# dedis/kyber

Measured on AMD Instinct MI355X. Metric: scalar-muls/s + pairings/s per node; MSM sec at 2^20 points, higher is better.
Workload: dtype int32 limbs (radix 2^25.5), int64 accumulate; 1 GPU; Ed25519 batched fixed-base + var-base scalar-mul, 2^20 scalars per GPU (BASELINE.json configs[1]); elements_per_gpu=1048576

## Files before the change

kyber_amd/csrc/ed25519.hip:

```cpp
#ifndef KYB_TU_WAVES
#define KYB_TU_WAVES 2
#endif
#include "context.h"
#include "ed25519_dev.cuh"
#include "msm.cuh"
#include "ed25519_h2c.cuh"
#include <stdlib.h>
#include <string.h>

#include <algorithm>
#include <atomic>
#include <chrono>
#include <thread>
#include <vector>

namespace kyb {


template <int G = 2>
__global__ void ed25519_build_base_table_kernel(int32_t* __restrict__ tab, const uint32_t* __restrict__ point,
                                                uint32_t* __restrict__ ok, int rows = ED_TAB_POS * ED_TAB_ENT) {
    const int t = blockIdx.x * blockDim.x + threadIdx.x;
    if (t >= rows) return;
    ge_p3 B;
    if (point) {
        uint32_t pw[8];
        load_words8(pw, point);
        const bool good = ge_p3_fromwords(B, pw);
        if (t == 0) *ok = good ? 1u : 0u;
    } else {
        B.X = fe_bx(); B.Y = fe_by(); fe_1(B.Z); B.T = fe_bt();
    }
    ed_comb_row<G>(tab + (size_t)t * ED_TAB_STRIDE, t, B);
}

__global__ __launch_bounds__(64, KYB_TU_WAVES) void ed25519_encode_kernel(size_t n, const int32_t* __restrict__ proj,
                                                            const uint8_t* __restrict__ status,
                                                            uint32_t* __restrict__ out) {
    ed_encode_chunk(n, proj, (size_t)blockIdx.x * blockDim.x + threadIdx.x, [&](size_t i, uint32_t (&w)[8]) {
        if (status && status[i]) {
#pragma unroll
            for (int k = 0; k < 8; k++) w[k] = 0;
        }
        store_words8(out + i * 8, w);
    });
}


template <int G>
__global__ __launch_bounds__(256, 3) void ed25519_mul_base_kernel(
    size_t n, const uint32_t* __restrict__ scalars, uint32_t* __restrict__ out,
    const int32_t* __restrict__ tab, uint32_t flags, int32_t* __restrict__ proj) {
    const bool full = (flags & KYB_F_VARTIME) != 0;
    for (size_t idx = (size_t)blockIdx.x * blockDim.x + threadIdx.x; idx < n;
         idx += (size_t)gridDim.x * blockDim.x) {
        uint32_t a[8];
        load_words8(a, scalars + idx * 8);
        int8_t e[65];
        recode16(e, a, full);
        ge_p3 h;
        ge_p3_0(h);
        ge_precomp t;
        ge_p1p1 r;
        const int npos = full ? EdComb<G>::POS : EdComb<G>::POS_CT;
#pragma unroll 1
        for (int k = 0; k < npos; k++) {
            int d = 0;
#pragma unroll
            for (int i = G - 1; i >= 0; i--)
                if (G * k + i <= 64) d = 16 * d + (int)e[G * k + i];
            if (full && __ballot(d != 0) == 0) continue;
            select_precomp_tab<EdComb<G>::ENT>(t, tab, k, d);
            ge_madd(r, h, t);
            ge_p1p1_to_p3(h, r);
        }
        if (proj) {
            store_proj(proj, idx, h);
            continue;
        }
        uint32_t w[8];
        ge_p3_towords(w, h);
        store_words8(out + idx * 8, w);
    }
}

KYB_DEV void select_precomp_uniform(ge_precomp& t, const int32_t* __restrict__ tab, int i, int b) {
    const bool neg = b < 0;
    const int babs = neg ? -b : b;
    const int pos = i >> 1, mult = (i & 1) ? 16 : 1;
    fe_1(t.ypx);
    fe_1(t.ymx);
    fe_0(t.xy2d);
#pragma unroll 1
    for (int m = 1; m <= 8; m++) {
        const int4* e = reinterpret_cast<const int4*>(tab + (size_t)(pos * ED_TAB_ENT + (m * mult - 1)) * ED_TAB_STRIDE);
        int32_t w[32];
#pragma unroll
        for (int q = 0; q < 8; q++) {
            const int4 x = e[q];
            w[4 * q] = x.x;
            w[4 * q + 1] = x.y;
            w[4 * q + 2] = x.z;
            w[4 * q + 3] = x.w;
        }
        const int32_t keep = -(int32_t)(babs == m);
#pragma unroll
        for (int l = 0; l < 10; l++) {
            t.ypx.v[l] ^= (t.ypx.v[l] ^ w[l]) & keep;
            t.ymx.v[l] ^= (t.ymx.v[l] ^ w[10 + l]) & keep;
            t.xy2d.v[l] ^= (t.xy2d.v[l] ^ w[20 + l]) & keep;
        }
    }
    ge_precomp_cneg(t, neg);
}
__global__ __launch_bounds__(256, 3) void ed25519_mul_base_uniform_kernel(
    size_t n, const uint32_t* __restrict__ scalars, uint32_t* __restrict__ out,
    const int32_t* __restrict__ tab, int32_t* __restrict__ proj) {
    for (size_t idx = (size_t)blockIdx.x * blockDim.x + threadIdx.x; idx < n;
         idx += (size_t)gridDim.x * blockDim.x) {
        uint32_t a[8];
        load_words8(a, scalars + idx * 8);
        int8_t e[65];
        recode16(e, a, false);
        ge_p3 h;
        ge_p3_0(h);
        ge_precomp t;
        ge_p1p1 r;
#pragma unroll 1
        for (int i = 0; i < 64; i++) {
            select_precomp_uniform(t, tab, i, (int)e[i]);
            ge_madd(r, h, t);
            ge_p1p1_to_p3(h, r);
        }
        if (proj) {
            store_proj(proj, idx, h);
            continue;
        }
        uint32_t w[8];
        ge_p3_towords(w, h);
        store_words8(out + idx * 8, w);
    }
}


template <bool GTAB, bool UNI = false>
__global__ __launch_bounds__(128, 3) void ed25519_mul_kernel(
    size_t n, const uint32_t* __restrict__ scalars, const uint32_t* __restrict__ points,
    size_t points_stride, uint32_t* __restrict__ out, uint8_t* __restrict__ status,
    uint32_t flags, int32_t* __restrict__ proj, int4* __restrict__ gtab) {
    const size_t idx = (size_t)blockIdx.x * blockDim.x + threadIdx.x;
    if (idx >= n) return;
    const bool full = !UNI && (flags & KYB_F_VARTIME) != 0;
    uint32_t pw[8], a[8];
    load_words8(pw, points + idx * points_stride);
    load_words8(a, scalars + idx * 8);
    ge_p3 A;
    const bool ok = ge_p3_fromwords(A, pw);
    int8_t e[65];
    recode16(e, a, full);
    ge_p3 h;
    const int vt_top = full ? wave_top_digit(a) : 63;
    if constexpr (GTAB) {
        TabGlobal tab{gtab + idx * 80};
        ge_scalarmult_w4<UNI>(h, e, A, full, tab, vt_top);
    } else {
        TabScratch tab;
        ge_scalarmult_w4<UNI>(h, e, A, full, tab, vt_top);
    }
    if (proj) {
        store_proj(proj, idx, h);
        if (status) status[idx] = ok ? KYB_ST_OK : KYB_ST_BAD_POINT;
        return;
    }
    uint32_t w[8];
    ge_p3_towords(w, h);
    if (!ok) {
#pragma unroll
        for (int i = 0; i < 8; i++) w[i] = 0;
    }
    store_words8(out + idx * 8, w);
    if (status) status[idx] = ok ? KYB_ST_OK : KYB_ST_BAD_POINT;
}

int ed25519_build_tables(DeviceCtx* ctx) {
    KYB_HIP_CHECK(hipMalloc(&ctx->ed_base_tab, ED_TAB_WORDS * sizeof(int32_t)));
    hipLaunchKernelGGL(ed25519_build_base_table_kernel<2>, dim3((ED_TAB_POS * ED_TAB_ENT + 63) / 64), dim3(64), 0,
                       nullptr, ctx->ed_base_tab, (const uint32_t*)nullptr, (uint32_t*)nullptr, ED_TAB_POS * ED_TAB_ENT);
    KYB_HIP_CHECK(hipGetLastError());
    const auto t0 = std::chrono::steady_clock::now();
    KYB_HIP_CHECK(hipMalloc(&ctx->ed_wide_tab, ED_WIDE_WORDS * sizeof(int32_t)));
    hipLaunchKernelGGL(ed25519_build_base_table_kernel<ED_COMB_G>, dim3((EdWide::ROWS + 63) / 64), dim3(64), 0, nullptr,
                       ctx->ed_wide_tab, (const uint32_t*)nullptr, (uint32_t*)nullptr, EdWide::ROWS);
    KYB_HIP_CHECK(hipGetLastError());
    KYB_HIP_CHECK(hipStreamSynchronize(nullptr));
    ctx->ed_wide_build_us = std::chrono::duration_cast<std::chrono::microseconds>(std::chrono::steady_clock::now() - t0).count();
    return KYB_OK;
}
void ed25519_free_tables(DeviceCtx* ctx) {
    if (ctx->ed_base_tab) hipFree(ctx->ed_base_tab);
    if (ctx->ed_wide_tab) hipFree(ctx->ed_wide_tab);
    ctx->ed_base_tab = ctx->ed_wide_tab = nullptr;
}

constexpr size_t ENC_DEFER_MIN = 4096;

static int ed_proj_workspace(DeviceCtx* ctx, hipStream_t st, size_t n, bool need_status, int32_t** proj,
                             uint8_t** status, int4** gtab = nullptr) {
    const size_t tab_bytes = gtab ? n * 1280 : 0;
    const size_t want = tab_bytes + n * 30 * sizeof(int32_t) + (need_status ? n : 0) + 256;
    void* base;
    int rc = ctx_workspace(ctx, WS_ED, st, want, &base);
    if (rc) return rc;
    if (gtab) *gtab = (int4*)base;
    *proj = (int32_t*)((uint8_t*)base + tab_bytes);
    if (status) *status = (uint8_t*)base + tab_bytes + n * 30 * sizeof(int32_t);
    return KYB_OK;
}

static int launch_mul_base(DeviceCtx* ctx, size_t n, const void* d_scalars, void* d_out, uint32_t flags,
                           hipStream_t st, const int32_t* tab = nullptr) {
    const bool wide = !tab && !(flags & KYB_F_UNIFORM);
    if (!tab) tab = wide ? ctx->ed_wide_tab : ctx->ed_base_tab;
    if (n == 0) return KYB_OK;
    const int block = 256;
    size_t want = (n + block - 1) / block;
    size_t cap = (size_t)ctx->num_cu * 8;
    int grid = (int)(want < cap ? want : cap);
    int32_t* proj = nullptr;
    std::lock_guard<std::recursive_mutex> enq_lock(ctx->enq_mu);
    if (n >= ENC_DEFER_MIN) {
        int rc = ed_proj_workspace(ctx, st, n, false, &proj, nullptr);
        if (rc) return rc;
    }
    if (flags & KYB_F_UNIFORM)
        hipLaunchKernelGGL(ed25519_mul_base_uniform_kernel, dim3(grid), dim3(block), 0, st, n,
                           (const uint32_t*)d_scalars, (uint32_t*)d_out, tab, proj);
    else if (wide)
        hipLaunchKernelGGL(ed25519_mul_base_kernel<ED_COMB_G>, dim3(grid), dim3(block), 0, st, n,
                           (const uint32_t*)d_scalars, (uint32_t*)d_out, tab, flags, proj);
    else
        hipLaunchKernelGGL(ed25519_mul_base_kernel<2>, dim3(grid), dim3(block), 0, st, n,
                           (const uint32_t*)d_scalars, (uint32_t*)d_out, tab, flags, proj);
    if (proj) {
        const size_t lanes = (n + ENC_CHUNK - 1) / ENC_CHUNK;
        hipLaunchKernelGGL(ed25519_encode_kernel, dim3((unsigned)((lanes + 63) / 64)), dim3(64), 0, st, n, proj,
                           (const uint8_t*)nullptr, (uint32_t*)d_out);
    }
    KYB_HIP_CHECK(hipGetLastError());
    return KYB_OK;
}
static int launch_mul(size_t n, const void* d_scalars, const void* d_points, size_t stride, void* d_out,
                      void* d_status, uint32_t flags, hipStream_t st) {
    if (n == 0) return KYB_OK;
    const int block = 128;
    size_t grid = (n + block - 1) / block;
    int32_t* proj = nullptr;
    int4* gtab = nullptr;
    uint8_t* stat = (uint8_t*)d_status;
    DeviceCtx* ctx;
    int rc = get_ctx(&ctx);
    if (rc) return rc;
    std::lock_guard<std::recursive_mutex> enq_lock(ctx->enq_mu);
    if (n >= ENC_DEFER_MIN) {
        rc = ed_proj_workspace(ctx, st, n, stat == nullptr, &proj, stat ? nullptr : &stat, &gtab);
        if (rc) return rc;
        if (flags & KYB_F_UNIFORM)
            hipLaunchKernelGGL((ed25519_mul_kernel<true, true>), dim3((unsigned)grid), dim3(block), 0, st, n,
                               (const uint32_t*)d_scalars, (const uint32_t*)d_points, stride, (uint32_t*)d_out, stat, flags,
                               proj, gtab);
        else
            hipLaunchKernelGGL(ed25519_mul_kernel<true>, dim3((unsigned)grid), dim3(block), 0, st, n,
                               (const uint32_t*)d_scalars, (const uint32_t*)d_points, stride, (uint32_t*)d_out, stat, flags,
                               proj, gtab);
    } else if (flags & KYB_F_UNIFORM) {
        hipLaunchKernelGGL((ed25519_mul_kernel<false, true>), dim3((unsigned)grid), dim3(block), 0, st, n,
                           (const uint32_t*)d_scalars, (const uint32_t*)d_points, stride, (uint32_t*)d_out, stat, flags,
                           proj, gtab);
    } else {
        hipLaunchKernelGGL(ed25519_mul_kernel<false>, dim3((unsigned)grid), dim3(block), 0, st, n,
                           (const uint32_t*)d_scalars, (const uint32_t*)d_points, stride, (uint32_t*)d_out, stat, flags,
                           proj, gtab);
    }
    if (proj) {
        const size_t lanes = (n + ENC_CHUNK - 1) / ENC_CHUNK;
        hipLaunchKernelGGL(ed25519_encode_kernel, dim3((unsigned)((lanes + 63) / 64)), dim3(64), 0, st, n, proj,
                           (const uint8_t*)stat, (uint32_t*)d_out);
    }
    KYB_HIP_CHECK(hipGetLastError());
    return KYB_OK;
}

}

using namespace kyb;

static bool ed_mul_flags_bad(uint32_t flags) {
    return (flags & ~(KYB_F_VARTIME | KYB_F_UNIFORM)) || (flags & (KYB_F_VARTIME | KYB_F_UNIFORM)) == (KYB_F_VARTIME | KYB_F_UNIFORM);
}

extern "C" {

int kyb_ed25519_mul_base_dev(size_t n, const void* d_scalars, void* d_out, uint32_t flags, void* stream) {
    if ((n && (!d_scalars || !d_out)) || ed_mul_flags_bad(flags)) {
        set_error("kyb_ed25519_mul_base_dev: bad argument");
        return KYB_E_ARG;
    }
    DeviceCtx* ctx;
    int rc = get_ctx(&ctx);
    if (rc) return rc;
    return launch_mul_base(ctx, n, d_scalars, d_out, flags, (hipStream_t)stream);
}

int kyb_ed25519_mul_dev(size_t n, const void* d_scalars, const void* d_points, void* d_out, void* d_status,
                        uint32_t flags, void* stream) {
    if ((n && (!d_scalars || !d_points || !d_out)) || ed_mul_flags_bad(flags)) {
        set_error("kyb_ed25519_mul_dev: bad argument");
        return KYB_E_ARG;
    }
    DeviceCtx* ctx;
    int rc = get_ctx(&ctx);
    if (rc) return rc;
    return launch_mul(n, d_scalars, d_points, 8, d_out, d_status, flags, (hipStream_t)stream);
}

static int mul_host(size_t n, const uint8_t* scalars, const uint8_t* points, size_t stride, uint8_t* out,
                    uint8_t* status, uint32_t flags);

int kyb_ed25519_mul_base(size_t n, const uint8_t* scalars, uint8_t* out, uint32_t flags) {
    if ((n && (!scalars || !out)) || ed_mul_flags_bad(flags)) {
        set_error("kyb_ed25519_mul_base: bad argument");
        return KYB_E_ARG;
    }
    if (n == 0) return KYB_OK;
    if (md_active(n))
        return md_run(n, [&](int, size_t lo, size_t hi) { return kyb_ed25519_mul_base(hi - lo, scalars + 32 * lo, out + 32 * lo, flags); });
    return mul_host(n, scalars, nullptr, 0, out, nullptr, flags);
}

constexpr size_t PIPE_CHUNK_MAX = PIN_SLOT_ELEMS;
constexpr int PIPE_SLOTS = DeviceCtx::NPIN, PIPE_STREAMS = 3;
static size_t pipe_chunk(const DeviceCtx* ctx) {
    if (const char* e = getenv("KYB_PIPE_CHUNK")) {
        const size_t v = (size_t)strtoull(e, nullptr, 10) & ~size_t(63);
        if (v >= 4096) return std::min(PIPE_CHUNK_MAX, v);
    }
    (void)ctx;
    return size_t(1) << 17;
}
static int pipe_nstreams() {
    if (const char* e = getenv("KYB_PIPE_STREAMS")) {
        const int v = atoi(e);
        if (v >= 1 && v <= PIPE_STREAMS) return v;
    }
    return 2;
}
constexpr size_t SAME_BASE_TABLE_MIN = 16384;

static int pipe_streams(DeviceCtx::StagePool* pool) {
    for (int i = 0; i < PIPE_STREAMS; i++)
        if (!pool->pipe[i]) KYB_HIP_CHECK(hipStreamCreateWithFlags(&pool->pipe[i], hipStreamNonBlocking));
    return KYB_OK;
}

static int mul_host(size_t n, const uint8_t* scalars, const uint8_t* points, size_t stride, uint8_t* out,
                    uint8_t* status, uint32_t flags) {
    DeviceCtx* ctx;
    int rc = get_ctx(&ctx);
    if (rc) return rc;
    bool fixed = points == nullptr;
    const size_t npts = fixed ? 0 : (stride ? n : 1);
    StageScope sc_(ctx);
    StageBuf d_s, d_p, d_o, d_st, d_tab;
    if ((rc = d_s.alloc(n * 32))) return rc;
    if ((rc = d_p.alloc(npts * 32))) return rc;
    if ((rc = d_o.alloc(n * 32))) return rc;
    if ((rc = d_st.alloc(n))) return rc;
    const int32_t* tab = nullptr;
    if (!fixed && !stride && (n >= SAME_BASE_TABLE_MIN || (flags & KYB_F_UNIFORM))) {
        if ((rc = d_tab.alloc(ED_TAB_WORDS * sizeof(int32_t) + 256))) return rc;
        uint32_t* d_ok = (uint32_t*)((uint8_t*)d_tab.p + ED_TAB_WORDS * sizeof(int32_t));
        KYB_HIP_CHECK(hipMemcpy(d_p.p, points, 32, hipMemcpyHostToDevice));
        hipLaunchKernelGGL(ed25519_build_base_table_kernel<2>, dim3((ED_TAB_POS * ED_TAB_ENT + 63) / 64), dim3(64), 0, sc_.stream(),
                           (int32_t*)d_tab.p, (const uint32_t*)d_p.p, d_ok, ED_TAB_POS * ED_TAB_ENT);
        uint32_t ok = 0;
        KYB_HIP_CHECK(hipMemcpy(&ok, d_ok, 4, hipMemcpyDeviceToHost));
        if (!ok) {
            memset(out, 0, n * 32);
            if (status) memset(status, KYB_ST_BAD_POINT, n);
            return KYB_OK;
        }
        if (status) memset(status, 0, n);
        tab = (const int32_t*)d_tab.p;
        fixed = true;
    }
    auto launch = [&](size_t off, size_t cnt, hipStream_t st) -> int {
        uint8_t* s = (uint8_t*)d_s.p + off * 32;
        uint8_t* o = (uint8_t*)d_o.p + off * 32;
        if (fixed) return launch_mul_base(ctx, cnt, s, o, flags, st, tab);
        const uint8_t* p = (const uint8_t*)d_p.p + (stride ? off * 32 : 0);
        return launch_mul(cnt, s, p, stride, o, (uint8_t*)d_st.p + off, flags, st);
    };
    const size_t PIPE_CHUNK = pipe_chunk(ctx);
    if (n < 2 * PIPE_CHUNK) {
        KYB_HIP_CHECK(hipMemcpy(d_s.p, scalars, n * 32, hipMemcpyHostToDevice));
        if (npts) KYB_HIP_CHECK(hipMemcpy(d_p.p, points, npts * 32, hipMemcpyHostToDevice));
        if ((rc = launch(0, n, nullptr))) return rc;
        if ((rc = d_o.download(out, n * 32))) return rc;
        if (status && !fixed) rc = d_st.download(status, n);
        return rc;
    }
    DeviceCtx::StagePool* pool = sc_.pool;
    if ((rc = pipe_streams(pool))) return rc;
    const int nstreams = pipe_nstreams();
    const bool per_point = !fixed && stride;
    const bool want_status = status && !fixed;
    if ((rc = ctx_pin_slots(pool))) return rc;
    const size_t nchunks = (n + PIPE_CHUNK - 1) / PIPE_CHUNK;
    std::vector<hipEvent_t> ev_out(nchunks);
    for (size_t i = 0; i < nchunks; i++) KYB_HIP_CHECK(hipEventCreateWithFlags(&ev_out[i], hipEventDisableTiming));
    auto enqueue = [&](size_t i) -> int {
        const size_t off = i * PIPE_CHUNK, cnt = std::min(PIPE_CHUNK, n - off);
        uint8_t* pin = (uint8_t*)pool->pin_in[i % PIPE_SLOTS];
        uint8_t* pout = (uint8_t*)pool->pin_out[i % PIPE_SLOTS];
        hipStream_t s_k = pool->pipe[i % nstreams];
        par_memcpy(pin, scalars + off * 32, cnt * 32);
        if (per_point) par_memcpy(pin + PIPE_CHUNK_MAX * 32, points + off * 32, cnt * 32);
        int r;
        if (fixed) {
            r = launch_mul_base(ctx, cnt, pin, pout, flags, s_k, tab);
        } else {
            const uint8_t* p = per_point ? pin + PIPE_CHUNK_MAX * 32 : (const uint8_t*)d_p.p;
            r = launch_mul(cnt, pin, p, stride, pout, (uint8_t*)d_st.p + off, flags, s_k);
        }
        if (r) return r;
        if (want_status)
            KYB_HIP_CHECK(hipMemcpyAsync(pout + PIPE_CHUNK_MAX * 32, (uint8_t*)d_st.p + off, cnt, hipMemcpyDeviceToHost, s_k));
        KYB_HIP_CHECK(hipEventRecord(ev_out[i], s_k));
        return KYB_OK;
    };
    auto drain = [&](size_t i) -> int {
        const size_t off = i * PIPE_CHUNK, cnt = std::min(PIPE_CHUNK, n - off);
        KYB_HIP_CHECK(hipEventSynchronize(ev_out[i]));
        const uint8_t* pout = (const uint8_t*)pool->pin_out[i % PIPE_SLOTS];
        par_memcpy(out + off * 32, pout, cnt * 32);
        if (want_status) memcpy(status + off, pout + PIPE_CHUNK_MAX * 32, cnt);
        return KYB_OK;
    };
    if (!fixed && !stride) KYB_HIP_CHECK(hipMemcpy(d_p.p, points, 32, hipMemcpyHostToDevice));
    std::atomic<size_t> enqueued{0}, drained{0};
    std::atomic<int> drain_rc{KYB_OK};
    std::atomic<bool> stop{false};
    const int device = ctx->device;
    std::string drain_err;
    std::thread drainer([&] {
        if (hipSetDevice(device) != hipSuccess) {
            drain_err = "ed25519 host pipeline: hipSetDevice failed on the drain thread";
            drain_rc.store(KYB_E_HIP);
            return;
        }
        for (size_t i = 0; i < nchunks; i++) {
            while (enqueued.load(std::memory_order_acquire) <= i) {
                if (stop.load(std::memory_order_acquire)) return;
                std::this_thread::yield();
            }
            const int r = drain(i);
            if (r) {
                drain_err = kyb_last_error();
                drain_rc.store(r);
                return;
            }
            drained.store(i + 1, std::memory_order_release);
        }
    });
    for (size_t i = 0; i < nchunks && rc == KYB_OK; i++) {
        while (i >= (size_t)PIPE_SLOTS && drained.load(std::memory_order_acquire) + PIPE_SLOTS <= i && drain_rc.load() == KYB_OK)
            std::this_thread::yield();
        if (drain_rc.load() != KYB_OK) break;
        rc = enqueue(i);
        if (rc == KYB_OK) enqueued.store(i + 1, std::memory_order_release);
    }
    if (rc != KYB_OK) stop.store(true, std::memory_order_release);
    drainer.join();
    if (rc == KYB_OK && (rc = drain_rc.load()) != KYB_OK) set_error(drain_err);
    hipError_t e2 = hipSuccess;
    for (int i = 0; i < PIPE_STREAMS; i++) {
        const hipError_t e = hipStreamSynchronize(pool->pipe[i]);
        if (e != hipSuccess) e2 = e;
    }
    for (size_t i = 0; i < nchunks; i++) hipEventDestroy(ev_out[i]);
    if (rc == KYB_OK && e2 != hipSuccess) {
        set_error("ed25519 host pipeline: stream synchronisation failed");
        rc = KYB_E_HIP;
    }
    return rc;
}

int kyb_ed25519_mul(size_t n, const uint8_t* scalars, const uint8_t* points, uint8_t* out, uint8_t* status,
                    uint32_t flags) {
    if ((n && (!scalars || !points || !out)) || ed_mul_flags_bad(flags)) {
        set_error("kyb_ed25519_mul: bad argument");
        return KYB_E_ARG;
    }
    if (n == 0) return KYB_OK;
    if (md_active(n))
        return md_run(n, [&](int, size_t lo, size_t hi) {
            return kyb_ed25519_mul(hi - lo, scalars + 32 * lo, points + 32 * lo, out + 32 * lo, status ? status + lo : nullptr, flags);
        });
    return mul_host(n, scalars, points, 8, out, status, flags);
}

int kyb_ed25519_mul_same_base(size_t n, const uint8_t* scalars, const uint8_t point[32], uint8_t* out,
                              uint8_t* status, uint32_t flags) {
    if ((n && (!scalars || !out)) || !point || ed_mul_flags_bad(flags)) {
        set_error("kyb_ed25519_mul_same_base: bad argument");
        return KYB_E_ARG;
    }
    if (n == 0) return KYB_OK;
    if (md_active(n))
        return md_run(n, [&](int, size_t lo, size_t hi) {
            return kyb_ed25519_mul_same_base(hi - lo, scalars + 32 * lo, point, out + 32 * lo, status ? status + lo : nullptr, flags);
        });
    return mul_host(n, scalars, point, 0, out, status, flags);
}

int kyb_ed25519_debug_base_table(int32_t* out) {
    if (!out) return KYB_E_ARG;
    DeviceCtx* ctx;
    int rc = get_ctx(&ctx);
    if (rc) return rc;
    KYB_HIP_CHECK(hipMemcpy(out, ctx->ed_base_tab, ED_TAB_WORDS * sizeof(int32_t), hipMemcpyDeviceToHost));
    return KYB_OK;
}

int kyb_ed25519_comb_info(int64_t info[6]) {
    if (!info) return KYB_E_ARG;
    DeviceCtx* ctx;
    int rc = get_ctx(&ctx);
    if (rc) return rc;
    info[0] = ED_COMB_G;
    info[1] = EdWide::POS;
    info[2] = EdWide::ENT;
    info[3] = EdWide::LAST_ENT;
    info[4] = (int64_t)(ED_WIDE_WORDS * sizeof(int32_t));
    info[5] = ctx->ed_wide_build_us;
    return KYB_OK;
}

int kyb_ed25519_debug_comb_table(int pos, int row0, int nrows, int32_t* out) {
    if (!out || pos < 0 || pos >= EdWide::POS || row0 < 0 || nrows < 0 ||
        row0 + nrows > (pos == EdWide::POS - 1 ? EdWide::LAST_ENT : EdWide::ENT)) {
        set_error("kyb_ed25519_debug_comb_table: bad argument");
        return KYB_E_ARG;
    }
    DeviceCtx* ctx;
    int rc = get_ctx(&ctx);
    if (rc) return rc;
    const size_t off = ((size_t)pos * EdWide::ENT + row0) * ED_TAB_STRIDE;
    KYB_HIP_CHECK(hipMemcpy(out, ctx->ed_wide_tab + off, (size_t)nrows * ED_TAB_STRIDE * sizeof(int32_t), hipMemcpyDeviceToHost));
    return KYB_OK;
}
}

namespace kyb {
struct EdMsm {
    using Aff = ge_precomp;
    using Acc = ge_p3;
    static constexpr int WIRE = 32, OUT = 32;
    static constexpr bool SCALAR_BE = false;
    static constexpr uint32_t COMBINE_FLAGS = 0;
    static constexpr int DECODE_WAVES = 3;
    __host__ __device__ static size_t wire_size(uint32_t) { return 32; }
    __device__ static int decode(Aff& a, const uint8_t* wire, uint32_t) {
        uint32_t w[8];
        load_words8(w, reinterpret_cast<const uint32_t*>(wire));
        ge_p3 p;
        const bool ok = ge_p3_fromwords(p, w);
        fe one;
        fe_1(one);
        fe_add(a.ypx, p.Y, p.X);
        fe_sub(a.ymx, p.Y, p.X);
        fe_mul(a.ypx, a.ypx, one);
        fe_mul(a.ymx, a.ymx, one);
        fe_mul(a.xy2d, p.T, fe_d2());
        return ok ? KYB_ST_OK : KYB_ST_BAD_POINT;
    }
    __device__ static void scalar_words(uint32_t (&k)[8], const uint8_t* wire) {
        load_words8(k, reinterpret_cast<const uint32_t*>(wire));
    }
    static constexpr bool HAS_EFFECTIVE = true;
// ... 246 lines not shown
```

kyber_amd/csrc/ed25519_dev.cuh:

```cuda
#pragma once
#include "ge25519.cuh"

#if !defined(__HIPCC__)
#include <type_traits>
struct int4 { int32_t x, y, z, w; };
struct uint4 { uint32_t x, y, z, w; };
inline int4 make_int4(int32_t x, int32_t y, int32_t z, int32_t w) { return int4{x, y, z, w}; }
inline uint4 make_uint4(uint32_t x, uint32_t y, uint32_t z, uint32_t w) { return uint4{x, y, z, w}; }
#define KYB_DEV_CONST static
#else
#define KYB_DEV_CONST __device__
#endif

namespace kyb {

constexpr int ED_TAB_POS = 33;
constexpr int ED_TAB_ENT = 136;
constexpr int ED_TAB_STRIDE = 32;
constexpr int ED_TAB_WORDS = ED_TAB_POS * ED_TAB_ENT * ED_TAB_STRIDE;

template <int G>
struct EdComb {
    static constexpr int POS = (65 + G - 1) / G;
    static constexpr int POS_CT = (64 + G - 1) / G;
    static constexpr int ENT = 8 * ((1 << (4 * G)) - 1) / 15;
    static constexpr int LAST_D = 65 - G * (POS - 1);
    static constexpr int LAST_ENT = 8 * ((1 << (4 * LAST_D)) - 1) / 15;
    static constexpr int ROWS = (POS - 1) * ENT + LAST_ENT;
};
#ifndef ED_COMB_G
#define ED_COMB_G 4
#endif
using EdWide = EdComb<ED_COMB_G>;
constexpr size_t ED_WIDE_WORDS = (size_t)EdWide::ROWS * ED_TAB_STRIDE;

KYB_DEV void load_words8(uint32_t w[8], const uint32_t* __restrict__ p) {
    const uint4 a = reinterpret_cast<const uint4*>(p)[0];
    const uint4 b = reinterpret_cast<const uint4*>(p)[1];
    w[0] = a.x; w[1] = a.y; w[2] = a.z; w[3] = a.w;
    w[4] = b.x; w[5] = b.y; w[6] = b.z; w[7] = b.w;
}
KYB_DEV void store_words8(uint32_t* __restrict__ p, const uint32_t w[8]) {
    reinterpret_cast<uint4*>(p)[0] = make_uint4(w[0], w[1], w[2], w[3]);
    reinterpret_cast<uint4*>(p)[1] = make_uint4(w[4], w[5], w[6], w[7]);
}

template <int G>
KYB_DEV void ed_comb_row(int32_t* __restrict__ o, int t, const ge_p3& B) {
    constexpr int ENT = EdComb<G>::ENT;
    const int pos = t / ENT, j = t - pos * ENT;
    ge_cached cB;
    ge_p3_to_cached(cB, B);
    ge_p3 acc;
    ge_p3_0(acc);
    ge_p1p1 r;
#pragma unroll 1
    for (int bit = 4 * G - 1; bit >= 0; bit--) {
        ge_dbl(r, acc.X, acc.Y, acc.Z);
        ge_p1p1_to_p3(acc, r);
        if (((j + 1) >> bit) & 1) {
            ge_add(r, acc, cB);
            ge_p1p1_to_p3(acc, r);
        }
    }
#pragma unroll 1
    for (int k = 0; k < 4 * G * pos; k++) {
        ge_dbl(r, acc.X, acc.Y, acc.Z);
        ge_p1p1_to_p3(acc, r);
    }
    fe zi, x, y, ypx, ymx, xy2d, z;
    fe_invert(zi, acc.Z);
    fe_mul(x, acc.X, zi);
    fe_mul(y, acc.Y, zi);
    fe_add(ypx, y, x);
    fe_sub(ymx, y, x);
    fe_mul(xy2d, x, y);
    fe_mul(xy2d, xy2d, fe_d2());
    fe_1(z);
    fe_mul(ypx, ypx, z);
    fe_mul(ymx, ymx, z);
#pragma unroll
    for (int l = 0; l < 10; l++) {
        o[l] = ypx.v[l];
        o[10 + l] = ymx.v[l];
        o[20 + l] = xy2d.v[l];
    }
    o[30] = o[31] = 0;
}

constexpr int ENC_CHUNK = 16;

KYB_DEV void store_proj(int32_t* __restrict__ proj, size_t idx, const ge_p3& h) {
    int32_t* o = proj + idx * 30;
#pragma unroll
    for (int l = 0; l < 10; l++) {
        o[l] = h.X.v[l];
        o[10 + l] = h.Y.v[l];
        o[20 + l] = h.Z.v[l];
    }
}
KYB_DEV void load_fe(fe& f, const int32_t* __restrict__ p) {
#pragma unroll
    for (int l = 0; l < 10; l++) f.v[l] = p[l];
}
template <class Emit>
KYB_DEV void ed_encode_chunk(size_t n, const int32_t* __restrict__ proj, size_t lane, Emit emit) {
    const size_t lo = lane * ENC_CHUNK;
    if (lo >= n) return;
    const int cnt = (int)((n - lo) < (size_t)ENC_CHUNK ? (n - lo) : (size_t)ENC_CHUNK);
    fe pre[ENC_CHUNK];
    fe z, acc;
    load_fe(acc, proj + lo * 30 + 20);
    pre[0] = acc;
#pragma unroll 1
    for (int j = 1; j < cnt; j++) {
        load_fe(z, proj + (lo + j) * 30 + 20);
        fe_mul(acc, acc, z);
        pre[j] = acc;
    }
    fe inv;
    fe_invert(inv, acc);
#pragma unroll 1
    for (int j = cnt - 1; j >= 0; j--) {
        fe zi, X, Y;
        load_fe(z, proj + (lo + j) * 30 + 20);
        if (j > 0) {
            fe_mul(zi, inv, pre[j - 1]);
            fe_mul(inv, inv, z);
        } else {
            zi = inv;
        }
        load_fe(X, proj + (lo + j) * 30);
        load_fe(Y, proj + (lo + j) * 30 + 10);
        uint32_t w[8];
        ge_encode_with_zinv(w, X, Y, zi);
        emit(lo + j, w);
    }
}

template <int ENT>
KYB_DEV void select_precomp_tab(ge_precomp& t, const int32_t* __restrict__ tab, int pos, int b) {
    const bool neg = b < 0;
    const int babs = neg ? -b : b;
    const int4* e = reinterpret_cast<const int4*>(tab + (size_t)(pos * ENT + (babs ? babs - 1 : 0)) * ED_TAB_STRIDE);
    int32_t w[32];
#pragma unroll
    for (int i = 0; i < 8; i++) {
        const int4 x = e[i];
        w[4 * i] = x.x;
        w[4 * i + 1] = x.y;
        w[4 * i + 2] = x.z;
        w[4 * i + 3] = x.w;
    }
#pragma unroll
    for (int l = 0; l < 10; l++) {
        t.ypx.v[l] = w[l];
        t.ymx.v[l] = w[10 + l];
        t.xy2d.v[l] = w[20 + l];
    }
    if (babs == 0) {
        fe_1(t.ypx);
        fe_1(t.ymx);
        fe_0(t.xy2d);
    }
    ge_precomp_cneg(t, neg);
}

struct TabScratch {
    ge_cached tab[8];
    KYB_DEV void put(int j, const ge_cached& c) { tab[j] = c; }
    KYB_DEV void get(ge_cached& c, int j) const { c = tab[j]; }
};
struct TabGlobal {
    int4* base;
    KYB_DEV void put(int j, const ge_cached& c) {
        int4* q = base + j * 10;
        const fe* f[4] = {&c.YpX, &c.YmX, &c.Z, &c.T2d};
        int32_t w[40];
#pragma unroll
        for (int k = 0; k < 4; k++)
#pragma unroll
            for (int l = 0; l < 10; l++) w[10 * k + l] = f[k]->v[l];
#pragma unroll
        for (int i = 0; i < 10; i++) q[i] = make_int4(w[4 * i], w[4 * i + 1], w[4 * i + 2], w[4 * i + 3]);
    }
    KYB_DEV void get(ge_cached& c, int j) const {
        const int4* q = base + j * 10;
        int32_t w[40];
#pragma unroll
        for (int i = 0; i < 10; i++) {
            const int4 x = q[i];
            w[4 * i] = x.x;
            w[4 * i + 1] = x.y;
            w[4 * i + 2] = x.z;
            w[4 * i + 3] = x.w;
        }
        fe* f[4] = {&c.YpX, &c.YmX, &c.Z, &c.T2d};
#pragma unroll
        for (int k = 0; k < 4; k++)
#pragma unroll
            for (int l = 0; l < 10; l++) f[k]->v[l] = w[10 * k + l];
    }
    KYB_DEV void get_signed(ge_cached& c, int b) const;
};
KYB_DEV_CONST __attribute__((aligned(16))) const int32_t ED_CACHED_IDENTITY[40] = {1, 0, 0, 0, 0, 0, 0, 0, 0, 0,
                                                                               1, 0, 0, 0, 0, 0, 0, 0, 0, 0,
                                                                               1};
KYB_DEV void TabGlobal::get_signed(ge_cached& c, int b) const {
    const bool neg = b < 0;
    const int babs = neg ? -b : b;
#if defined(__HIPCC__)
    typedef int32_t i32x2 __attribute__((ext_vector_type(2)));
    typedef int32_t i32x4 __attribute__((ext_vector_type(4)));
    using gint = const __attribute__((address_space(1))) int32_t;
    using gint2 = const __attribute__((address_space(1))) i32x2;
    using gint4 = const __attribute__((address_space(1))) i32x4;
#else
    struct i32x2 { int32_t x, y; };
    struct i32x4 { int32_t x, y, z, w; };
    using gint = const int32_t;
    using gint2 = const i32x2;
    using gint4 = const i32x4;
#endif
    gint* e = babs ? (gint*)(base + (babs - 1) * 10) : (gint*)ED_CACHED_IDENTITY;
    gint2* p = (gint2*)(e + (neg ? 10 : 0));
    gint2* m = (gint2*)(e + (neg ? 0 : 10));
    gint4* q = (gint4*)(e + 20);
#pragma unroll
    for (int i = 0; i < 5; i++) {
        const i32x2 x = p[i], y = m[i];
        c.YpX.v[2 * i] = x.x;
        c.YpX.v[2 * i + 1] = x.y;
        c.YmX.v[2 * i] = y.x;
        c.YmX.v[2 * i + 1] = y.y;
    }
    int32_t w[20];
#pragma unroll
    for (int i = 0; i < 5; i++) {
        const i32x4 x = q[i];
        w[4 * i] = x.x;
        w[4 * i + 1] = x.y;
        w[4 * i + 2] = x.z;
        w[4 * i + 3] = x.w;
    }
    const int32_t s = -(int32_t)neg;
#pragma unroll
    for (int l = 0; l < 10; l++) {
        c.Z.v[l] = w[l];
        c.T2d.v[l] = (w[10 + l] ^ s) - s;
    }
}
template <bool UNI = false, class Tab>
KYB_DEV void select_cached(ge_cached& c, const Tab& tab, int b) {
    const bool neg = b < 0;
    const int babs = neg ? -b : b;
    if constexpr (UNI) {
        ge_cached_0(c);
#pragma unroll 1
        for (int m = 1; m <= 8; m++) {
            ge_cached x;
            tab.get(x, m - 1);
            const int32_t keep = -(int32_t)(babs == m);
#pragma unroll
            for (int l = 0; l < 10; l++) {
                c.YpX.v[l] ^= (c.YpX.v[l] ^ x.YpX.v[l]) & keep;
                c.YmX.v[l] ^= (c.YmX.v[l] ^ x.YmX.v[l]) & keep;
                c.Z.v[l] ^= (c.Z.v[l] ^ x.Z.v[l]) & keep;
                c.T2d.v[l] ^= (c.T2d.v[l] ^ x.T2d.v[l]) & keep;
            }
        }
    } else if constexpr (std::is_same_v<Tab, TabGlobal>) {
        tab.get_signed(c, b);
        return;
    } else {
        tab.get(c, babs ? babs - 1 : 0);
        if (babs == 0) ge_cached_0(c);
    }
    ge_cached_cneg(c, neg);
}

KYB_DEV int wave_top_digit(const uint32_t a[8]) {
    int bits = 0;
#pragma unroll
    for (int i = 0; i < 8; i++)
        if (a[i]) bits = 32 * i + 32 - __builtin_clz(a[i]);
    int t = (bits + 3) >> 2;
    if (t > 64) t = 64;
#if defined(__HIP_DEVICE_COMPILE__)
#pragma unroll
    for (int off = 32; off >= 1; off >>= 1) {
        const int o = __shfl_xor(t, off, 64);
        t = o > t ? o : t;
    }
    t = __builtin_amdgcn_readfirstlane(t);
#endif
    return t;
}

template <class Tab>
KYB_DEV void ge_window_table(Tab& tab, const ge_p3& A) {
    ge_p1p1 t;
    ge_p3 u;
    ge_cached c;
    ge_p3_to_cached(c, A);
    tab.put(0, c);
#pragma unroll 1
    for (int i = 0; i < 7; i++) {
        ge_add(t, A, c);
        ge_p1p1_to_p3(u, t);
        ge_p3_to_cached(c, u);
        tab.put(i + 1, c);
    }
}

template <bool UNI = false, class Tab>
KYB_DEV void ge_scalarmult_w4(ge_p3& h, const int8_t e[65], const ge_p3& A, bool full, Tab& tab, int vt_top) {
    ge_p1p1 t;
    ge_p3 u;
    ge_p2 r;
    ge_cached c;
    ge_window_table(tab, A);
    ge_p3_0(u);
    int top = 63;
    if (full) top = vt_top;
    select_cached<UNI>(c, tab, e[top]);
    ge_add(t, u, c);
    uint32_t pk[8];
#pragma unroll
    for (int j = 0; j < 8; j++) {
        pk[j] = 0;
#pragma unroll
        for (int q = 0; q < 8; q++) pk[j] |= (uint32_t)((e[8 * j + q] + 8) & 15) << (4 * q);
    }
    auto shl4 = [&pk]() {
#pragma unroll
        for (int j = 7; j > 0; j--) pk[j] = (pk[j] << 4) | (pk[j - 1] >> 28);
        pk[0] <<= 4;
    };
#pragma unroll 1
    for (int i = top; i < 64; i++) shl4();
#pragma unroll 1
    for (int i = top - 1; i >= 0; i--) {
        const int d = (int)(pk[7] >> 28) - 8;
        shl4();
        ge_p1p1_to_p2(r, t);
        ge_dbl(t, r.X, r.Y, r.Z);
        ge_p1p1_to_p2(r, t);
        ge_dbl(t, r.X, r.Y, r.Z);
        ge_p1p1_to_p2(r, t);
        ge_dbl(t, r.X, r.Y, r.Z);
        ge_p1p1_to_p2(r, t);
        ge_dbl(t, r.X, r.Y, r.Z);
#if defined(__HIP_DEVICE_COMPILE__)
        if (!UNI && full && __ballot(d != 0) == 0) continue;
#endif
        ge_p1p1_to_p3(u, t);
        select_cached<UNI>(c, tab, d);
        ge_add(t, u, c);
    }
    ge_p1p1_to_p3(h, t);
}

}
```

kyber_amd/csrc/ge25519.cuh:

```cuda
#pragma once
#include "fe25519.cuh"

namespace kyb {

struct ge_p2 { fe X, Y, Z; };
struct ge_p3 { fe X, Y, Z, T; };
struct ge_p1p1 { fe X, Y, Z, T; };
struct ge_cached { fe YpX, YmX, Z, T2d; };
struct ge_precomp { fe ypx, ymx, xy2d; };

#include "ed25519_consts.inc"

KYB_DEV void ge_p3_0(ge_p3& h) {
    fe_0(h.X);
    fe_1(h.Y);
    fe_1(h.Z);
    fe_0(h.T);
}
KYB_DEV void ge_cached_0(ge_cached& c) {
    fe_1(c.YpX);
    fe_1(c.YmX);
    fe_1(c.Z);
    fe_0(c.T2d);
}
KYB_DEV void ge_p1p1_to_p2(ge_p2& r, const ge_p1p1& p) {
    fe_mul(r.X, p.X, p.T);
    fe_mul(r.Y, p.Y, p.Z);
    fe_mul(r.Z, p.Z, p.T);
}
KYB_DEV void ge_p1p1_to_p3(ge_p3& r, const ge_p1p1& p) {
    fe_mul(r.X, p.X, p.T);
    fe_mul(r.Y, p.Y, p.Z);
    fe_mul(r.Z, p.Z, p.T);
    fe_mul(r.T, p.X, p.Y);
}
KYB_DEV void ge_p3_to_cached(ge_cached& r, const ge_p3& p) {
    fe_add(r.YpX, p.Y, p.X);
    fe_sub(r.YmX, p.Y, p.X);
    r.Z = p.Z;
    fe_mul(r.T2d, p.T, fe_d2());
}
KYB_DEV void ge_dbl(ge_p1p1& r, const fe& X, const fe& Y, const fe& Z) {
    fe t0;
    fe_sq(r.X, X);
    fe_sq(r.Z, Y);
    fe_sq2(r.T, Z);
    fe_add(r.Y, X, Y);
    fe_sq(t0, r.Y);
    fe_add(r.Y, r.Z, r.X);
    fe_sub(r.Z, r.Z, r.X);
    fe_sub(r.X, t0, r.Y);
    fe_sub(r.T, r.T, r.Z);
}
KYB_DEV void ge_add(ge_p1p1& r, const ge_p3& p, const ge_cached& q) {
    fe t0;
    fe_add(r.X, p.Y, p.X);
    fe_sub(r.Y, p.Y, p.X);
    fe_mul(r.Z, r.X, q.YpX);
    fe_mul(r.Y, r.Y, q.YmX);
    fe_mul(r.T, q.T2d, p.T);
    fe_mul(r.X, p.Z, q.Z);
    fe_add(t0, r.X, r.X);
    fe_sub(r.X, r.Z, r.Y);
    fe_add(r.Y, r.Z, r.Y);
    fe_add(r.Z, t0, r.T);
    fe_sub(r.T, t0, r.T);
}
KYB_DEV void ge_madd(ge_p1p1& r, const ge_p3& p, const ge_precomp& q) {
    fe t0;
    fe_add(r.X, p.Y, p.X);
    fe_sub(r.Y, p.Y, p.X);
    fe_mul(r.Z, r.X, q.ypx);
    fe_mul(r.Y, r.Y, q.ymx);
    fe_mul(r.T, q.xy2d, p.T);
    fe_add(t0, p.Z, p.Z);
    fe_sub(r.X, r.Z, r.Y);
    fe_add(r.Y, r.Z, r.Y);
    fe_add(r.Z, t0, r.T);
    fe_sub(r.T, t0, r.T);
}
KYB_DEV void ge_cached_cneg(ge_cached& c, bool neg) {
    fe_cswap(c.YpX, c.YmX, neg);
    fe nt;
    fe_neg(nt, c.T2d);
    fe_cmov(c.T2d, nt, neg);
}
KYB_DEV void ge_precomp_cneg(ge_precomp& c, bool neg) {
    fe_cswap(c.ypx, c.ymx, neg);
    fe nt;
    fe_neg(nt, c.xy2d);
    fe_cmov(c.xy2d, nt, neg);
}

KYB_DEV void ge_encode_with_zinv(uint32_t w[8], const fe& X, const fe& Y, const fe& zinv) {
    fe x, y;
    fe_mul(x, X, zinv);
    fe_mul(y, Y, zinv);
    fe_towords(w, y);
    w[7] ^= (uint32_t)fe_isnegative(x) << 31;
}
KYB_DEV void ge_p3_towords(uint32_t w[8], const ge_p3& p) {
    fe zi;
    fe_invert(zi, p.Z);
    ge_encode_with_zinv(w, p.X, p.Y, zi);
}
KYB_DEV bool ge_p3_fromwords(ge_p3& p, const uint32_t w[8]) {
    fe u, v, v3, vxx, check;
    fe_fromwords(p.Y, w);
    fe_1(p.Z);
    fe_sq(u, p.Y);
    fe_mul(v, u, fe_d());
    fe_sub(u, u, p.Z);
    fe_add(v, v, p.Z);
    fe_sq(v3, v);
    fe_mul(v3, v3, v);
    fe_sq(p.X, v3);
    fe_mul(p.X, p.X, v);
    fe_mul(p.X, p.X, u);
    fe_pow22523(p.X, p.X);
    fe_mul(p.X, p.X, v3);
    fe_mul(p.X, p.X, u);
    fe_sq(vxx, p.X);
    fe_mul(vxx, vxx, v);
    fe_sub(check, vxx, u);
    bool ok = true;
    if (fe_isnonzero(check)) {
        fe_add(check, vxx, u);
        ok = !fe_isnonzero(check);
        fe xs;
        fe_mul(xs, p.X, fe_sqrtm1());
        p.X = xs;
    }
    const bool sign = (w[7] >> 31) != 0;
    fe nx;
    fe_neg(nx, p.X);
    fe_cmov(p.X, nx, fe_isnegative(p.X) != sign);
    fe_mul(p.T, p.X, p.Y);
    return ok;
}

KYB_DEV void recode16(int8_t e[65], const uint32_t a[8], bool full256) {
    int carry = 0;
#pragma unroll
    for (int i = 0; i < 64; i++) {
        int d = (int)((a[i >> 3] >> ((i & 7) * 4)) & 15) + carry;
        if (i < 63) {
            carry = (d + 8) >> 4;
            d -= carry << 4;
        }
        e[i] = (int8_t)d;
    }
    int top = e[63];
    int c2 = 0;
    if (full256) {
        c2 = (top + 8) >> 4;
        top -= c2 << 4;
    } else if (top > 8) {
        top = 0;
    }
    e[63] = (int8_t)top;
    e[64] = (int8_t)c2;
}

KYB_DEV bool ed_effective_scalar(uint32_t (&k)[8]) {
    uint32_t c = 0, t7 = 0;
#pragma unroll
    for (int j = 0; j < 8; j++) {
        const uint64_t s = (uint64_t)k[j] + (j < 7 ? 0x88888888u : 0x08888888u) + c;
        t7 = (uint32_t)s;
        c = (uint32_t)(s >> 32);
    }
    const uint32_t e63 = (c << 4) | (t7 >> 28);
    if (e63 <= 8) return false;
    const uint32_t carried = e63 - (k[7] >> 28);
    k[7] &= 0x0fffffffu;
    if (!carried) return false;
    uint32_t b = 0;
#pragma unroll
    for (int j = 0; j < 8; j++) {
        const uint64_t d = (uint64_t)(j == 7 ? 0x10000000u : 0u) - k[j] - b;
        k[j] = (uint32_t)d;
        b = (uint32_t)(d >> 63);
    }
    return true;
}

}
```

Measured before the change: 171.7 million scalar-muls/s.

## Replace Fermat inversion in batched encode with safegcd divsteps inversion

Adds a Bernstein-Yang style divsteps modular inverse using 30-bit limbs with batches of 30 steps. It replaces the exponentiation-based fe_invert in the batched-encode chunk. A fixed-iteration variant is used for uniform (constant-time) calls and a variable-time early-exit loop otherwise. The encode kernel's chunk size is kept at 16 through a new template parameter, while the global ENC_CHUNK default drops to 8. The aim is to cut the per-chunk inversion cost, at the price of a noinline call and int64-heavy arithmetic on the GPU.

Result: no change. 172.5 million scalar-muls/s (median of 6 runs) (+0.5%).

```diff
diff --git a/kyber_amd/csrc/ed25519.hip b/kyber_amd/csrc/ed25519.hip
--- a/kyber_amd/csrc/ed25519.hip
+++ b/kyber_amd/csrc/ed25519.hip
@@ -34,16 +34,27 @@
     ed_comb_row<G>(tab + (size_t)t * ED_TAB_STRIDE, t, B);
 }
 
+constexpr int ENC_CHUNK_MUL = 16;
+template <bool UNI>
+KYB_DEV void ed_encode_store(size_t n, const int32_t* __restrict__ proj, const uint8_t* __restrict__ status,
+                             uint32_t* __restrict__ out) {
+    ed_encode_chunk<ENC_CHUNK_MUL, UNI>(n, proj, (size_t)blockIdx.x * blockDim.x + threadIdx.x, [&](size_t i, uint32_t (&w)[8]) {
+        if (status && status[i]) {
+#pragma unroll
+            for (int k = 0; k < 8; k++) w[k] = 0;
+        }
+        store_words8(out + i * 8, w);
+    });
+}
 __global__ __launch_bounds__(64, KYB_TU_WAVES) void ed25519_encode_kernel(size_t n, const int32_t* __restrict__ proj,
                                                             const uint8_t* __restrict__ status,
                                                             uint32_t* __restrict__ out) {
-    ed_encode_chunk(n, proj, (size_t)blockIdx.x * blockDim.x + threadIdx.x, [&](size_t i, uint32_t (&w)[8]) {
-        if (status && status[i]) {
-#pragma unroll
-            for (int k = 0; k < 8; k++) w[k] = 0;
-        }
-        store_words8(out + i * 8, w);
-    });
+    ed_encode_store<false>(n, proj, status, out);
+}
+__global__ __launch_bounds__(64, KYB_TU_WAVES) void ed25519_uniform_encode_kernel(size_t n, const int32_t* __restrict__ proj,
+                                                                    const uint8_t* __restrict__ status,
+                                                                    uint32_t* __restrict__ out) {
+    ed_encode_store<true>(n, proj, status, out);
 }
 
 
@@ -217,6 +228,16 @@
     return KYB_OK;
 }
 
+static void launch_encode(size_t n, const int32_t* proj, const uint8_t* status, uint32_t* out, uint32_t flags,
+                          hipStream_t st) {
+    const size_t lanes = (n + ENC_CHUNK_MUL - 1) / ENC_CHUNK_MUL;
+    const dim3 grid((unsigned)((lanes + 63) / 64));
+    if (flags & KYB_F_UNIFORM)
+        hipLaunchKernelGGL(ed25519_uniform_encode_kernel, grid, dim3(64), 0, st, n, proj, status, out);
+    else
+        hipLaunchKernelGGL(ed25519_encode_kernel, grid, dim3(64), 0, st, n, proj, status, out);
+}
+
 static int launch_mul_base(DeviceCtx* ctx, size_t n, const void* d_scalars, void* d_out, uint32_t flags,
                            hipStream_t st, const int32_t* tab = nullptr) {
     const bool wide = !tab && !(flags & KYB_F_UNIFORM);
@@ -242,9 +263,7 @@
         hipLaunchKernelGGL(ed25519_mul_base_kernel<2>, dim3(grid), dim3(block), 0, st, n,
                            (const uint32_t*)d_scalars, (uint32_t*)d_out, tab, flags, proj);
     if (proj) {
-        const size_t lanes = (n + ENC_CHUNK - 1) / ENC_CHUNK;
-        hipLaunchKernelGGL(ed25519_encode_kernel, dim3((unsigned)((lanes + 63) / 64)), dim3(64), 0, st, n, proj,
-                           (const uint8_t*)nullptr, (uint32_t*)d_out);
+        launch_encode(n, proj, nullptr, (uint32_t*)d_out, flags, st);
     }
     KYB_HIP_CHECK(hipGetLastError());
     return KYB_OK;
@@ -282,9 +301,7 @@
                            proj, gtab);
     }
     if (proj) {
-        const size_t lanes = (n + ENC_CHUNK - 1) / ENC_CHUNK;
-        hipLaunchKernelGGL(ed25519_encode_kernel, dim3((unsigned)((lanes + 63) / 64)), dim3(64), 0, st, n, proj,
-                           (const uint8_t*)stat, (uint32_t*)d_out);
+        launch_encode(n, proj, stat, (uint32_t*)d_out, flags, st);
     }
     KYB_HIP_CHECK(hipGetLastError());
     return KYB_OK;
diff --git a/kyber_amd/csrc/ed25519_dev.cuh b/kyber_amd/csrc/ed25519_dev.cuh
--- a/kyber_amd/csrc/ed25519_dev.cuh
+++ b/kyber_amd/csrc/ed25519_dev.cuh
@@ -88,7 +88,10 @@
     o[30] = o[31] = 0;
 }
 
-constexpr int ENC_CHUNK = 16;
+#ifndef KYB_ENC_CHUNK
+#define KYB_ENC_CHUNK 8
+#endif
+constexpr int ENC_CHUNK = KYB_ENC_CHUNK;
 
 KYB_DEV void store_proj(int32_t* __restrict__ proj, size_t idx, const ge_p3& h) {
     int32_t* o = proj + idx * 30;
@@ -103,12 +106,12 @@
 #pragma unroll
     for (int l = 0; l < 10; l++) f.v[l] = p[l];
 }
-template <class Emit>
+template <int CHUNK = ENC_CHUNK, bool UNI = false, class Emit>
 KYB_DEV void ed_encode_chunk(size_t n, const int32_t* __restrict__ proj, size_t lane, Emit emit) {
-    const size_t lo = lane * ENC_CHUNK;
+    const size_t lo = lane * CHUNK;
     if (lo >= n) return;
-    const int cnt = (int)((n - lo) < (size_t)ENC_CHUNK ? (n - lo) : (size_t)ENC_CHUNK);
-    fe pre[ENC_CHUNK];
+    const int cnt = (int)((n - lo) < (size_t)CHUNK ? (n - lo) : (size_t)CHUNK);
+    fe pre[CHUNK];
     fe z, acc;
     load_fe(acc, proj + lo * 30 + 20);
     pre[0] = acc;
@@ -119,7 +122,7 @@
         pre[j] = acc;
     }
     fe inv;
-    fe_invert(inv, acc);
+    fe_invert_divsteps<UNI>(inv, acc);
 #pragma unroll 1
     for (int j = cnt - 1; j >= 0; j--) {
         fe zi, X, Y;
diff --git a/kyber_amd/csrc/fe25519_inv.cuh b/kyber_amd/csrc/fe25519_inv.cuh
--- /dev/null
+++ b/kyber_amd/csrc/fe25519_inv.cuh
@@ -0,0 +1,142 @@
+#pragma once
+#include "fe25519.cuh"
+
+#if defined(__HIPCC__)
+#define KYB_DEV_NOINLINE __device__ __noinline__ inline
+#else
+#define KYB_DEV_NOINLINE inline
+#endif
+
+namespace kyb {
+
+constexpr int FE_INV_NL = 9;
+constexpr int FE_INV_FIXED_BATCHES = 25;
+constexpr uint32_t FE_INV_M30 = (1u << 30) - 1;
+KYB_DEV constexpr int32_t fe_inv_plimb(int i) {
+    return i == 0 ? (int32_t)((1u << 30) - 19) : i < FE_INV_NL - 1 ? (int32_t)FE_INV_M30 : (int32_t)((1u << 15) - 1);
+}
+constexpr uint32_t fe_inv_pinv() {
+    uint32_t x = 0u - 19u;
+    for (int k = 0; k < 5; k++) x *= 2u - (0u - 19u) * x;
+    return x;
+}
+
+template <bool FIXED = false>
+KYB_DEV_NOINLINE void fe_invert_divsteps(fe& out, const fe& z, int* batches = nullptr) {
+    constexpr int NL = FE_INV_NL;
+    constexpr uint32_t M30 = FE_INV_M30;
+    constexpr uint32_t PINV = fe_inv_pinv();
+    static_assert((uint32_t)(PINV * (0u - 19u)) == 1u, "p^-1 mod 2^32");
+    uint32_t w[8];
+    fe_towords(w, z);
+    int32_t f[NL], g[NL], d[NL], e[NL];
+#pragma unroll
+    for (int i = 0; i < NL; i++) {
+        const int bit = 30 * i, idx = bit >> 5, sh = bit & 31;
+        uint32_t x = w[idx] >> sh;
+        if (sh > 2 && idx + 1 < 8) x |= w[idx + 1] << (32 - sh);
+        g[i] = (int32_t)(x & M30);
+        f[i] = fe_inv_plimb(i);
+        d[i] = 0;
+        e[i] = 0;
+    }
+    e[0] = 1;
+    int32_t eta = -1;
+    uint32_t gnz = 0;
+#pragma unroll
+    for (int i = 0; i < NL; i++) gnz |= (uint32_t)g[i];
+    int nb = 0;
+#pragma unroll 1
+    while (FIXED ? nb < FE_INV_FIXED_BATCHES : gnz != 0) {
+        nb++;
+        uint32_t f0 = (uint32_t)f[0] | ((uint32_t)f[1] << 30), g0 = (uint32_t)g[0] | ((uint32_t)g[1] << 30);
+        uint32_t u = 1, v = 0, q = 0, rr = 1;
+#pragma unroll 6
+        for (int k = 0; k < 30; k++) {
+            const uint32_t c1 = (uint32_t)(eta >> 31);
+            const uint32_t c2 = 0u - (g0 & 1u);
+            const uint32_t x = (f0 ^ c1) - c1, y = (u ^ c1) - c1, t = (v ^ c1) - c1;
+            g0 += x & c2;
+            q += y & c2;
+            rr += t & c2;
+            const uint32_t sw = c1 & c2;
+            eta = (int32_t)(((uint32_t)eta ^ sw) - 1u);
+            f0 += g0 & sw;
+            u += q & sw;
+            v += rr & sw;
+            g0 >>= 1;
+            u <<= 1;
+            v <<= 1;
+        }
+        const int32_t U = (int32_t)u, V = (int32_t)v, Q = (int32_t)q, R = (int32_t)rr;
+        {
+            int64_t cf = (int64_t)U * f[0] + (int64_t)V * g[0], cg = (int64_t)Q * f[0] + (int64_t)R * g[0];
+            cf >>= 30;
+            cg >>= 30;
+#pragma unroll
+            for (int i = 1; i < NL; i++) {
+                cf += (int64_t)U * f[i] + (int64_t)V * g[i];
+                cg += (int64_t)Q * f[i] + (int64_t)R * g[i];
+                f[i - 1] = (int32_t)((uint32_t)cf & M30);
+                g[i - 1] = (int32_t)((uint32_t)cg & M30);
+                cf >>= 30;
+                cg >>= 30;
+            }
+            f[NL - 1] = (int32_t)cf;
+            g[NL - 1] = (int32_t)cg;
+        }
+        {
+            const int32_t sd = d[NL - 1] >> 31, se = e[NL - 1] >> 31;
+            int32_t md = (U & sd) + (V & se), me = (Q & sd) + (R & se);
+            int64_t cd = (int64_t)U * d[0] + (int64_t)V * e[0], ce = (int64_t)Q * d[0] + (int64_t)R * e[0];
+            md -= (int32_t)((PINV * (uint32_t)cd + (uint32_t)md) & M30);
+            me -= (int32_t)((PINV * (uint32_t)ce + (uint32_t)me) & M30);
+            cd -= (int64_t)19 * md;
+            ce -= (int64_t)19 * me;
+            cd >>= 30;
+            ce >>= 30;
+#pragma unroll
+            for (int i = 1; i < NL; i++) {
+                cd += (int64_t)U * d[i] + (int64_t)V * e[i];
+                ce += (int64_t)Q * d[i] + (int64_t)R * e[i];
+                if (i == NL - 1) {
+                    cd += (int64_t)md << 15;
+                    ce += (int64_t)me << 15;
+                }
+                d[i - 1] = (int32_t)((uint32_t)cd & M30);
+                e[i - 1] = (int32_t)((uint32_t)ce & M30);
+                cd >>= 30;
+                ce >>= 30;
+            }
+            d[NL - 1] = (int32_t)cd;
+            e[NL - 1] = (int32_t)ce;
+        }
+        gnz = 0;
+#pragma unroll
+        for (int i = 0; i < NL; i++) gnz |= (uint32_t)g[i];
+    }
+    if (batches) *batches = nb;
+    const int32_t sf = f[NL - 1] >> 31;
+#pragma unroll 1
+    for (int pass = 0; pass < 2; pass++) {
+        const int32_t neg = d[NL - 1] >> 31, s = pass ? 0 : sf;
+        int64_t c = 0;
+#pragma unroll
+        for (int i = 0; i < NL; i++) {
+            c += (int64_t)(((d[i] + (fe_inv_plimb(i) & neg)) ^ s) - s);
+            d[i] = i + 1 < NL ? (int32_t)((uint32_t)c & M30) : (int32_t)c;
+            if (i + 1 < NL) c >>= 30;
+        }
+    }
+#pragma unroll
+    for (int k = 0; k < 8; k++) {
+        const int bit = 32 * k, idx = bit / 30, sh = bit - 30 * idx;
+        uint32_t x = (uint32_t)d[idx] >> sh;
+        if (idx + 1 < NL) x |= (uint32_t)d[idx + 1] << (30 - sh);
+        if (60 - sh < 32 && idx + 2 < NL) x |= (uint32_t)d[idx + 2] << (60 - sh);
+        w[k] = x;
+    }
+    fe_fromwords(out, w);
+}
+
+}
diff --git a/kyber_amd/csrc/ge25519.cuh b/kyber_amd/csrc/ge25519.cuh
--- a/kyber_amd/csrc/ge25519.cuh
+++ b/kyber_amd/csrc/ge25519.cuh
@@ -1,5 +1,5 @@
 #pragma once
-#include "fe25519.cuh"
+#include "fe25519_inv.cuh"
 
 namespace kyb {
 
```
